# duckietown/gym-duckietown

Hardware: NVIDIA H100
Metric: env-steps/sec (obs+reward+done) at N envs, 1/2/4/8 H100 vs CPU ref (higher is better)
Workload: dtype f64 logic / f32 raster / u8 obs

## Files before the change

### gym-duckietown_b200/csrc/dts_render.cu

```cuda
#include <cstddef>

#include "dts_camera.cuh"
#include "dts_kernels.h"

namespace dts {

namespace {

#ifndef DTS_STATS
#define DTS_STATS 0
#endif
#if DTS_STATS
#define DTS_COUNT(slot, n) do { if (lane == 0) atomicAdd(err + (slot), (n)); } while (0)
#else
#define DTS_COUNT(slot, n) do { } while (0)
#endif
constexpr int kThreads = 256;
constexpr int kRasterMinCtas = 3;
constexpr int kSoloMinCtas = 3;
constexpr int kFlatMinCtas = 4;
constexpr int kGeoWarps = 1;
constexpr int kGeoMinCtas = 32;
constexpr int kWarps = kThreads / 32;
constexpr int kBinW = 8, kBinH = 4;
// ... 419 lines not shown
        if (e + lo < 0) inside &= ~(1u << f);
      }
    }
  }
  int tiny = 0;
  if (!fb && !quad && live) {
    const int minx = min(qx[0], min(qx[1], qx[2])) - ox, maxx = max(qx[0], max(qx[1], qx[2])) - ox;
    const int miny = min(qy[0], min(qy[1], qy[2])) - oy, maxy = max(qy[0], max(qy[1], qy[2])) - oy;
    const int x0 = max(minx >> 6, 0), x1 = min(maxx >> 6, kCoarseW - 1), y0 = max(miny >> 6, 0), y1 = min(maxy >> 6, kCoarseH - 1);
    if (x1 - x0 < 4 && y1 - y0 < 4 && x1 >= x0 && y1 >= y0) {
      tiny = kKindTiny;
      E0[3] = x0 | (y0 << 16); A[3] = x1 | (y1 << 16);
    }
  }
  const int id = __float_as_int(w2.w);
  int4* o = reinterpret_cast<int4*>(out);
  o[0] = make_int4(E0[0], E0[1], E0[2], E0[3]);
  o[1] = make_int4(A[0], A[1], A[2], A[3]);
  o[2] = make_int4(B[0], B[1], B[2], B[3]);
  o[3] = make_int4(__float_as_int(w2.x), __float_as_int(w2.y), __float_as_int(w2.z), id);
  o[4] = make_int4(qx[0] - ox, qy[0] - oy, (int)((unsigned)p | (live << 16) | ((inside & live) << 24)),
                   (quad ? kKindQuad : 0) | (id < 2 ? kKindGround : 0) | tiny | flat);
  return (inside & live) | (id < 2 ? kRecGround : 0u) | ((flat || id < 2) && !tiny ? kRecFlatOk : 0u);
}

struct ShadeIn {
  const PrimRec* pr;
  int x0, y0;
  float q0, qx, qy, u0, ux, uy, v0, vx, vy, r0;
  int ltq;
  unsigned tex;
};
__device__ __forceinline__ ShadeIn load_shade(const PrimRec* __restrict__ prims, unsigned w) {
  const PrimRec* pr = prims + w;
  const int2 xy0 = __ldg(reinterpret_cast<const int2*>(pr));
  const float4 w3 = __ldg(reinterpret_cast<const float4*>(pr) + 3);
  const float4 w4 = __ldg(reinterpret_cast<const float4*>(pr) + 4);
  const float4 w5 = __ldg(reinterpret_cast<const float4*>(pr) + 5);
  ShadeIn si;
  si.pr = pr; si.x0 = xy0.x; si.y0 = xy0.y;
  si.q0 = w3.x; si.qx = w3.y; si.qy = w3.z; si.u0 = w3.w;
  si.ux = w4.x; si.uy = w4.y; si.v0 = w4.z; si.vx = w4.w;
  si.vy = w5.x; si.ltq = __float_as_int(w5.y); si.tex = __float_as_uint(w5.z); si.r0 = w5.w;
  return si;
}
__device__ __forceinline__ void shade_eval(const ShadeIn& si, const uint8_t* __restrict__ tex_pool, const float4* __restrict__ lat_tab,
                                           int pxa, int pya, float c3[3]) {
  const float cdx = (float)(pxa + 32 - si.x0) * 0.015625f, cdy = (float)(pya + 32 - si.y0) * 0.015625f;
  float qq = fmaf(si.qy, cdy, fmaf(si.qx, cdx, si.q0));
  if (!(qq > 1e-20f)) qq = 1e-20f;
  const float rq = 1.0f / qq;
  const float u = fmaf(si.uy, cdy, fmaf(si.ux, cdx, si.u0)) * rq;
  const float v = fmaf(si.vy, cdy, fmaf(si.vx, cdx, si.v0)) * rq;
  const int ltq = si.ltq;
  const int lat = (ltq & 0xffff) - 1;
  if (lat >= 0) {
    const float fa_ = u * 7.0f, fb_ = (1.0f - v) * 7.0f;
    int ia = __float2int_rd(fa_), ib = __float2int_rd(fb_);
    ia = ia < 0 ? 0 : (ia > 6 ? 6 : ia);
    ib = ib < 0 ? 0 : (ib > 6 ? 6 : ib);
    const float fa = fa_ - (float)ia, fb = fb_ - (float)ib;
    const float4* L = lat_tab + lat * 64 + ia * 8 + ib;
    const bool lower = fb <= fa;
    const float4 c00 = L[0], c11 = L[9], cm = L[lower ? 8 : 1];
    const float t1 = lower ? fa : fb, t2 = lower ? fb : fa;
    c3[0] = fmaf(t2, c11.x - cm.x, fmaf(t1, cm.x - c00.x, c00.x));
    c3[1] = fmaf(t2, c11.y - cm.y, fmaf(t1, cm.y - c00.y, c00.y));
    c3[2] = fmaf(t2, c11.z - cm.z, fmaf(t1, cm.z - c00.z, c00.z));
  } else {
    const float4 w6 = __ldg(reinterpret_cast<const float4*>(si.pr) + 6);
    const float4 w7 = __ldg(reinterpret_cast<const float4*>(si.pr) + 7);
    c3[0] = fmaf(w6.y, cdy, fmaf(w6.x, cdx, si.r0)) * rq;
    c3[1] = fmaf(w7.x, cdy, fmaf(w6.w, cdx, w6.z)) * rq;
    c3[2] = fmaf(w7.w, cdy, fmaf(w7.z, cdx, w7.y)) * rq;
  }
  if (ltq & 0x00ff0000) {
    const unsigned ti = si.tex;
    const int lw = (ti >> 24) & 15, lh = ti >> 28;
    const int tw = 1 << lw, th = 1 << lh;
    const float twf = __int_as_float((127 + lw) << 23), thf = __int_as_float((127 + lh) << 23);
    const float tx = u * twf - 0.5f, ty = v * thf - 0.5f;
    const int txi = __float2int_rd(tx), tyi = __float2int_rd(ty);
    const float ffx = tx - (float)txi, ffy = ty - (float)tyi;
    const int ti0 = txi & (tw - 1), ti1 = (ti0 + 1) & (tw - 1);
    const int tj0 = tyi & (th - 1), tj1 = (tj0 + 1) & (th - 1);
    const uchar4* tp = reinterpret_cast<const uchar4*>(tex_pool + ((size_t)(ti & 0xffffffu) << 8));
    const uchar4 t00 = __ldg(tp + (tj0 << lw) + ti0), t10 = __ldg(tp + (tj0 << lw) + ti1);
    const uchar4 t01 = __ldg(tp + (tj1 << lw) + ti0), t11 = __ldg(tp + (tj1 << lw) + ti1);
    const float a0[3] = {(float)t00.x, (float)t00.y, (float)t00.z}, a1[3] = {(float)t10.x, (float)t10.y, (float)t10.z};
    const float b0[3] = {(float)t01.x, (float)t01.y, (float)t01.z}, b1[3] = {(float)t11.x, (float)t11.y, (float)t11.z};
#pragma unroll
    for (int ch = 0; ch < 3; ch++) {
      const float ta = fmaf(ffx, a1[ch] - a0[ch], a0[ch]);
      const float tb = fmaf(ffx, b1[ch] - b0[ch], b0[ch]);
      const float tc = fmaf(ffy, tb - ta, ta);
      c3[ch] = tc * (c3[ch] * 0.00392156862745098f);
    }
  }
}
__device__ __forceinline__ void shade_prim(const PrimRec* __restrict__ prims, unsigned w, const uint8_t* __restrict__ tex_pool,
                                           const float4* __restrict__ lat_tab, int pxa, int pya, float c3[3]) {
  const ShadeIn si = load_shade(prims, w);
  shade_eval(si, tex_pool, lat_tab, pxa, pya, c3);
}

__device__ __forceinline__ uint32_t smem_u32(const void* p) { return (uint32_t)__cvta_generic_to_shared(p); }
__device__ __forceinline__ void mbar_init(uint64_t* bar, int count) {
  asm volatile("mbarrier.init.shared::cta.b64 [%0], %1;" ::"r"(smem_u32(bar)), "r"(count) : "memory");
}
__device__ __forceinline__ void mbar_fence_init() {
  asm volatile("fence.mbarrier_init.release.cluster;" ::: "memory");
  asm volatile("fence.proxy.async.shared::cta;" ::: "memory");
}
__device__ __forceinline__ void mbar_expect_tx(uint64_t* bar, uint32_t bytes) {
  asm volatile("mbarrier.arrive.expect_tx.shared::cta.b64 _, [%0], %1;" ::"r"(smem_u32(bar)), "r"(bytes) : "memory");
}
__device__ __forceinline__ void bulk_load(void* dst_smem, const void* src_gmem, uint32_t bytes, uint64_t* bar) {
  asm volatile("cp.async.bulk.shared::cluster.global.mbarrier::complete_tx::bytes [%0], [%1], %2, [%3];" ::"r"(smem_u32(dst_smem)),
               "l"(src_gmem), "r"(bytes), "r"(smem_u32(bar))
               : "memory");
}
__device__ __forceinline__ void mbar_wait(uint64_t* bar, uint32_t parity) {
  uint32_t ok;
  do {
    asm volatile("{\n .reg .pred p;\n mbarrier.try_wait.parity.shared::cta.b64 p, [%1], %2;\n selp.u32 %0, 1, 0, p;\n}"
                 : "=r"(ok)
                 : "r"(smem_u32(bar)), "r"(parity)
                 : "memory");
  } while (!ok);
}

__device__ __forceinline__ unsigned pack_rgb(float r, float g, float b) {
  const unsigned ur = min(__float2uint_rn(r * 255.0f), 255u);
  const unsigned ug = min(__float2uint_rn(g * 255.0f), 255u);
  const unsigned ub = min(__float2uint_rn(b * 255.0f), 255u);
  return ur | (ug << 8) | (ub << 16);
}

struct StoreLane {
  int src_lo, src_hi;
  int sh8;
  int off;
  int j, row;
};
__device__ __forceinline__ StoreLane make_store_lane(int lane, int W) {
  StoreLane sl;
  const int j = lane & 7, rowbase = lane & ~7;
  const int p0 = (4 * j) / 3;
  sl.sh8 = (4 * j - 3 * p0) * 8;
  sl.src_lo = rowbase + min(p0, 7);
  sl.src_hi = rowbase + min(p0 + 1, 7);
  sl.off = (lane >> 3) * W * 3 + 4 * j;
  sl.j = j; sl.row = lane >> 3;
  return sl;
}
__device__ __forceinline__ void store_bin_fast(uint8_t* __restrict__ bin0, const StoreLane& sl, unsigned rgb, int rows_ok) {
  const unsigned lo = __shfl_sync(0xffffffffu, rgb, sl.src_lo);
  const unsigned hi = __shfl_sync(0xffffffffu, rgb, sl.src_hi);
  const unsigned word = __funnelshift_r(lo | (hi << 24), hi >> 8, sl.sh8);
  if (sl.j < 6 && sl.row < rows_ok) *reinterpret_cast<unsigned*>(bin0 + sl.off) = word;
}
__device__ __forceinline__ void store_bin(uint8_t* __restrict__ out, unsigned rgb, int lane, int bx, int by, int W, int H) {
  const int gx = bx * kBinW + (lane & 7), gy = by * kBinH + (lane >> 3);
  if ((W & 3) == 0 && bx * kBinW + kBinW <= W) {
    const int j = lane & 7, rowbase = lane & ~7;
    const int p0 = (4 * j) / 3, sh8 = (4 * j - 3 * p0) * 8;
    const unsigned lo = __shfl_sync(0xffffffffu, rgb, rowbase + min(p0, 7));
    const unsigned hi = __shfl_sync(0xffffffffu, rgb, rowbase + min(p0 + 1, 7));
    const unsigned long long both = (unsigned long long)lo | ((unsigned long long)hi << 24);
    if (j < 6 && gy < H)
      *reinterpret_cast<unsigned*>(out + ((size_t)gy * W + bx * kBinW) * 3 + 4 * j) = (unsigned)(both >> sh8);
// ... 559 lines not shown
        const int slot = atomicAdd(fm.work + kWorkSoloList, 1);
        fm.solo[slot] = make_uint2((unsigned)env, (unsigned)b | ((unsigned)p << 16));
        atomicOr(&no_flat[b], 1);
      }
      if (!(r & kRecFlatOk)) atomicOr(&no_flat[b], 1);
    }
  }
  if (!lean_fmt) return;
  __syncthreads();
  for (int b0 = wib * 32; b0 < cbins; b0 += nthr) {
    const int b = b0 + lane, c = b < cbins ? (cnt[b] & kCountMask) : 0;
    const bool flat = c >= 1 && c <= kStage && !no_flat[b];
    const unsigned m = __ballot_sync(0xffffffffu, flat);
    if (!m) continue;
    int base = 0;
    if (lane == 0) base = atomicAdd(fm.work + kWorkFlatList, __popc(m));
    base = __shfl_sync(0xffffffffu, base, 0);
    if (flat) {
      fm.bin_count[(size_t)env * cbins + b] = kFlatBin;
      fm.flat[base + __popc(m & ((1u << lane) - 1u))] = make_uint2((unsigned)env, (unsigned)b | ((unsigned)c << 16));
    }
  }
}

__device__ __noinline__ void emit_general(uint8_t* __restrict__ out, const GatherTab& gt, int n_peers, size_t env_off, int out_fmt,
                                          unsigned rgb, int lane, int bx, int by, int W, int H) {
  store_bin_any(out, out_fmt, rgb, lane, bx, by, W, H);
  for (int p = 0; p < n_peers; p++) store_bin_any(gt.base[p] + env_off, out_fmt, rgb, lane, bx, by, W, H);
}
__device__ __noinline__ void gather_rows_out(const uint8_t* __restrict__ src, const GatherTab& gt, size_t off, size_t nbytes, int lane) {
  __syncwarp();
  const uint8_t* s = src + off;
  if (((reinterpret_cast<size_t>(s) | nbytes) & 15) == 0) {
    bool aligned = true;
    for (int p = 0; p < gt.n; p++) aligned &= (reinterpret_cast<size_t>(gt.base[p] + off) & 15) == 0;
    if (aligned) {
      for (size_t i = (size_t)lane * 16; i < nbytes; i += 512) {
        const int4 v = __ldcg(reinterpret_cast<const int4*>(s + i));
        for (int p = 0; p < gt.n; p++) *reinterpret_cast<int4*>(gt.base[p] + off + i) = v;
      }
      return;
    }
  }
  for (size_t i = lane; i < nbytes; i += 32) {
    const uint8_t v = __ldcg(s + i);
    for (int p = 0; p < gt.n; p++) gt.base[p][off + i] = v;
  }
}

constexpr size_t kRasterSmem = (sizeof(BinRec) * 2 * kStage + 16 + 128 * sizeof(unsigned long long)) * kWarps;
__device__ __forceinline__ unsigned float_key(float f) { const unsigned b = __float_as_uint(f); return b ^ ((b >> 31) ? 0xffffffffu : 0x80000000u); }
__device__ __forceinline__ float key_float(unsigned k) { return __uint_as_float(k ^ ((k >> 31) ? 0x80000000u : 0xffffffffu)); }

__device__ __forceinline__ int sample_mask(const BinRec& br, int pxc, int pyc) {
  const int4 E = *reinterpret_cast<const int4*>(br.E0);
  const int4 A = *reinterpret_cast<const int4*>(br.A);
  const int4 B = *reinterpret_cast<const int4*>(br.B);
  const int ec0 = E.x + A.x * pxc + B.x * pyc;
  const int ec1 = E.y + A.y * pxc + B.y * pyc;
  const int ec2 = E.z + A.z * pxc + B.z * pyc;
  int mask = 0;
  if (br.kind & kKindQuad) {
    const int ec3 = E.w + A.w * pxc + B.w * pyc;
#pragma unroll
    for (int s = 0; s < 4; s++) {
      const int e0 = ec0 + A.x * sample_x(s) + B.x * sample_y(s);
      const int e1 = ec1 + A.y * sample_x(s) + B.y * sample_y(s);
      const int e2 = ec2 + A.z * sample_x(s) + B.z * sample_y(s);
      const int e3 = ec3 + A.w * sample_x(s) + B.w * sample_y(s);
      if ((e0 | e1 | e2 | e3) >= 0) mask |= 1 << s;
    }
  } else {
#pragma unroll
    for (int s = 0; s < 4; s++) {
      const int e0 = ec0 + A.x * sample_x(s) + B.x * sample_y(s);
      const int e1 = ec1 + A.y * sample_x(s) + B.y * sample_y(s);
      const int e2 = ec2 + A.z * sample_x(s) + B.z * sample_y(s);
      if ((e0 | e1 | e2) >= 0) mask |= 1 << s;
    }
  }
  return mask;
}

__device__ __forceinline__ unsigned shade_resolve(const unsigned wn[4], bool simple, const float clr[3], const PrimRec* __restrict__ prims,
                                                  const uint8_t* __restrict__ tex_pool, const float4* __restrict__ lat_tab, int pxa,
                                                  int pya, int lane, int32_t* __restrict__ err) {
  (void)lane; (void)err;
  const bool same = wn[1] == wn[0] && wn[2] == wn[0] && wn[3] == wn[0];
  const bool all_same = simple || __all_sync(0xffffffffu, same);
  float c3[3] = {clr[0], clr[1], clr[2]};
  if (wn[0] != kNoPrim) shade_prim(prims, wn[0], tex_pool, lat_tab, pxa, pya, c3);
  if (all_same) return pack_rgb(c3[0], c3[1], c3[2]);
  float s01[3] = {c3[0], c3[1], c3[2]}, s23[3] = {0.f, 0.f, 0.f};
  unsigned pend = 0xeu;
  if (wn[1] == wn[0]) { pend &= ~2u; s01[0] = s01[0] + c3[0]; s01[1] = s01[1] + c3[1]; s01[2] = s01[2] + c3[2]; }
#pragma unroll
  for (int t = 2; t < 4; t++)
    if (wn[t] == wn[0]) { pend &= ~(1u << t); s23[0] = s23[0] + c3[0]; s23[1] = s23[1] + c3[1]; s23[2] = s23[2] + c3[2]; }
#pragma unroll 1
  while (__any_sync(0xffffffffu, pend != 0u)) {
    DTS_COUNT(12, 1);
    if (pend) {
      const int s = __ffs(pend) - 1;
      const unsigned w = s == 1 ? wn[1] : (s == 2 ? wn[2] : wn[3]);
      float d3[3] = {clr[0], clr[1], clr[2]};
      if (w != kNoPrim) shade_prim(prims, w, tex_pool, lat_tab, pxa, pya, d3);
#pragma unroll
      for (int t = 1; t < 4; t++)
        if ((pend >> t & 1u) && wn[t] == w) {
          pend &= ~(1u << t);
          if (t < 2) { s01[0] = s01[0] + d3[0]; s01[1] = s01[1] + d3[1]; s01[2] = s01[2] + d3[2]; }
          else { s23[0] = s23[0] + d3[0]; s23[1] = s23[1] + d3[1]; s23[2] = s23[2] + d3[2]; }
        }
    }
  }
  return pack_rgb((s01[0] + s23[0]) * 0.25f, (s01[1] + s23[1]) * 0.25f, (s01[2] + s23[2]) * 0.25f);
}

template <bool kWrapFmt, bool kFish>
__global__ void __launch_bounds__(kThreads, kRasterMinCtas)
k_raster(const DState S, const DMap* __restrict__ maps, RenderCfg rc, FrameMem fm, FishTab ft, GatherTab gt,
         uint8_t* __restrict__ obs, int max_prims, int max_pairs, int max_lat, int32_t* __restrict__ err) {
  extern __shared__ __align__(128) unsigned char raster_smem[];
  BinRec (*stages)[2][kStage] = reinterpret_cast<BinRec (*)[2][kStage]>(raster_smem);
  uint64_t (*bars)[2] = reinterpret_cast<uint64_t (*)[2]>(raster_smem + sizeof(BinRec) * kWarps * 2 * kStage);
  unsigned long long* zb = reinterpret_cast<unsigned long long*>(raster_smem + sizeof(BinRec) * kWarps * 2 * kStage + 16 * kWarps) +
                           128 * (threadIdx.x >> 5);
  const int W = rc.width, H = rc.height;
  const int cbins_x = (W + kCoarseW - 1) / kCoarseW, cbins_y = (H + kCoarseH - 1) / kCoarseH, cbins = cbins_x * cbins_y;
  const int lane = threadIdx.x & 31, warp = threadIdx.x >> 5;
  const size_t frame_bytes = (size_t)W * H * 3;
  const int out_fmt = !kWrapFmt ? 0 : (rc.obs_layout | (rc.obs_dtype << 2));
  const size_t out_elem = (kWrapFmt && rc.obs_dtype == DTS_OBS_F32_UNIT) ? 4 : 1;
  const int pxs = (lane & 7) * kSub, pys = (lane >> 3) * kSub;
  const StoreLane sl = make_store_lane(lane, W);
  const bool fast_fmt = !kWrapFmt && lean_output(DTS_OBS_HWC, DTS_OBS_U8, W);
  const bool planar_u8 = kWrapFmt && rc.obs_dtype == DTS_OBS_U8 &&
                         ((rc.obs_layout == DTS_OBS_CHW && (W & 3) == 0) || (rc.obs_layout == DTS_OBS_CWH && (H & 3) == 0));
  uint64_t* bar = bars[warp];
  if (lane == 0) { mbar_init(&bar[0], 1); mbar_init(&bar[1], 1); mbar_fence_init(); }
  __syncwarp();
  uint32_t parity = 0;
  int cs = 0, ps = 0;
  const int n_work = rc.n_envs * cbins_y;
  int work = 0;
  if (lane == 0) work = atomicAdd(fm.work + kWorkRaster, 1);
  work = __shfl_sync(0xffffffffu, work, 0);
  while (work < n_work) {
    int next_work = 0;
    if (lane == 0) next_work = atomicAdd(fm.work + kWorkRaster, 1);
    const int env = work / cbins_y, cby = work - env * cbins_y;
    const DMap& m = maps[S.map_id[env]];
    const uint8_t* tex_pool = m.tex_pool;
    const PrimRec* prims = fm.prims + (size_t)env * max_prims;
    const BinRec* recs = fm.recs;
    const float4* lat_tab = fm.lat + (size_t)env * max_lat * 64;
    const size_t env_off = (size_t)env * frame_bytes * out_elem;
    uint8_t* out = obs + env_off;
    const bool gather_rows = gt.n > 0 && !kWrapFmt;
    auto emit = [&](unsigned rgb, int bx, int by) {
      if (fast_fmt && (gt.n == 0 || gather_rows) && bx * kBinW + kBinW <= W) {
        store_bin_fast(out + ((size_t)(by * kBinH) * W + bx * kBinW) * 3, sl, rgb, min(kBinH, H - by * kBinH));
      } else if (kWrapFmt && gt.n == 0) {
        if (planar_u8 && bx * kBinW + kBinW <= W && by * kBinH + kBinH <= H) {
          store_bin_planar_u8(out, out_fmt & 3, rgb, lane, bx, by, W, H);
        } else {
          const int gx = bx * kBinW + (lane & 7), gy = by * kBinH + (lane >> 3);
          if (gx < W && gy < H) store_px_fmt(out, out_fmt & 3, out_fmt >> 2, gx, gy, W, H, rgb);
        }
      } else {
        emit_general(out, gt, gather_rows ? 0 : gt.n, env_off, out_fmt, rgb, lane, bx, by, W, H);
      }
    };
    float clr[3];
    clear_colour(S, rc, env, clr);
    const unsigned clear_rgb = pack_rgb(clr[0], clr[1], clr[2]);
    int my_cnt = 0, my_start = 0;
    if (lane < cbins_x) {
      my_cnt = fm.bin_count[(size_t)env * cbins + cby * cbins_x + lane];
      my_start = fm.bin_start[(size_t)env * cbins + cby * cbins_x + lane];
    }
    const unsigned nz = __ballot_sync(0xffffffffu, my_cnt > 0);
    int pcbx = nz ? __ffs(nz) - 1 : 32, pf = 0, pc = 0;
    const unsigned rows_in = fine_rows_in_image(cby, H);
    auto fine_valid = [&](int cbx, int f) -> bool { return (fine_in_image(cbx, rows_in, W) >> f) & 1u; };
    auto next_bin = [&]() {
      const unsigned rem = nz & ~((2u << pcbx) - 1u);
      pcbx = rem ? __ffs(rem) - 1 : 32;
      pf = 0; pc = 0;
    };
    auto issue = [&]() {
      if (pcbx >= 32) return;
      const int n = __shfl_sync(0xffffffffu, my_cnt, pcbx), st = __shfl_sync(0xffffffffu, my_start, pcbx);
      if (n > kStage) while (pf < kCFX * kCFY && !fine_valid(pcbx, pf)) pf++;
      if (n > kStage && pf >= kCFX * kCFY) { next_bin(); return; }
      const int nch = min(kStage, n - pc);
      if (lane == 0) {
        mbar_expect_tx(&bar[ps], (uint32_t)(nch * sizeof(BinRec)));
        bulk_load(stages[warp][ps], recs + st + pc, (uint32_t)(nch * sizeof(BinRec)), &bar[ps]);
// ... 189 lines not shown
                      const int e0 = ec0 + A.x * sample_x(s) + B.x * sample_y(s);
                      const int e1 = ec1 + A.y * sample_x(s) + B.y * sample_y(s);
                      const int e2 = ec2 + A.z * sample_x(s) + B.z * sample_y(s);
                      if ((e0 | e1 | e2) < 0) continue;
                      const float sdx = (float)(X + sample_x(s) - xy0.x) * 0.015625f, sdy = (float)(Y + sample_y(s) - xy0.y) * 0.015625f;
                      const float zs = fmaf(zp.z, sdy, fmaf(zp.y, sdx, zp.x));
                      atomicMin(&zb[((py - fy0) * kBinW + (px - fx0)) * 4 + s], ((unsigned long long)float_key(zs) << 32) | tail);
                    }
                  }
              }
              __syncwarp();
            }
            if (!(last || simple)) continue;
            if (!kFish && !simple && zb_used) {
#pragma unroll
              for (int s = 0; s < 4; s++) {
                const unsigned long long k = zb[lane * 4 + s];
                if (k == ~0ull) continue;
                const float zt = key_float((unsigned)(k >> 32));
                bool win = zt < z[s];
                if (zt == z[s] && wn[s] != kNoPrim) win = (int)((k >> 16) & 0xffffu) < __ldg(&prims[wn[s]].id);
                if (win) { z[s] = zt; wn[s] = (unsigned)(k & 0xffffu); }
              }
              __syncwarp();
            }
            DTS_COUNT(11, 1);
            unsigned rgb = shade_resolve(wn, simple, clr, prims, tex_pool, lat_tab, ox + pxc, oy + pyc, lane, err);
            if (kFish && !px_valid) rgb = 0u;
            emit(rgb, bx, by);
          }
        }
      }
    }
    if (gather_rows) {
      const int rows = min(kCoarseH, H - cby * kCoarseH);
      gather_rows_out(obs, gt, env_off + (size_t)cby * kCoarseH * W * 3, (size_t)rows * W * 3, lane);
    }
    work = __shfl_sync(0xffffffffu, next_work, 0);
  }
}

template <bool kFish>
__global__ void __launch_bounds__(kThreads, kSoloMinCtas) k_raster_solo(const DState S, const DMap* __restrict__ maps, RenderCfg rc, FrameMem fm,
                                                                        FishTab ft, uint8_t* __restrict__ obs, int max_prims, int max_lat) {
  const int W = rc.width, H = rc.height;
  const int cbins_x = (W + kCoarseW - 1) / kCoarseW;
  const int lane = threadIdx.x & 31;
  const StoreLane sl = make_store_lane(lane, W);
  const size_t frame_bytes = (size_t)W * H * 3;
  const int n = fm.work[kWorkSoloList];
  const int warps = (gridDim.x * blockDim.x) >> 5;
  for (int i = (blockIdx.x * blockDim.x + threadIdx.x) >> 5; i < n; i += warps) {
    const uint2 e = fm.solo[i];
    const int env = (int)e.x, b = (int)(e.y & 0xffffu);
    const unsigned p = e.y >> 16;
    const int cby = b / cbins_x, cbx = b - cby * cbins_x;
    const uint8_t* tex_pool = maps[S.map_id[env]].tex_pool;
    const float4* lat_tab = fm.lat + (size_t)env * max_lat * 64;
    const ShadeIn si = load_shade(fm.prims + (size_t)env * max_prims, p);
    uint8_t* out = obs + (size_t)env * frame_bytes;
    const int nx = min(kCFX, (W - cbx * kCoarseW + kBinW - 1) / kBinW);
    const int ny = ((cby * kCFY + 1) * kBinH < H) ? 2 : 1;
#pragma unroll 1
    for (int fy = 0; fy < ny; fy++)
#pragma unroll 1
    for (int fx = 0; fx < nx; fx++) {
      const int bx = cbx * kCFX + fx, by = cby * kCFY + fy;
      int pxa = (bx * kBinW + (lane & 7)) * kSub, pya = (by * kBinH + (lane >> 3)) * kSub;
      bool px_valid = true;
      if (kFish) {
        const FishPx src = fish_source(ft, bx, by, lane, W, H);
        px_valid = src.valid;
        pxa = src.x; pya = src.y;
      }
      float c3[3];
      shade_eval(si, tex_pool, lat_tab, pxa, pya, c3);
      unsigned rgb = pack_rgb(c3[0], c3[1], c3[2]);
      if (kFish && !px_valid) rgb = 0u;
      store_bin_lean(out, sl, rgb, lane, bx, by, W, H);
    }
  }
}

template <bool kFish>
__global__ void __launch_bounds__(kThreads, kFlatMinCtas) k_raster_flat(const DState S, const DMap* __restrict__ maps, RenderCfg rc, FrameMem fm,
                                                                        FishTab ft, uint8_t* __restrict__ obs, int max_prims, int max_lat,
                                                                        int32_t* __restrict__ err) {
  __shared__ BinRec stages[kWarps][kStage];
  const int W = rc.width, H = rc.height;
  const int cbins_x = (W + kCoarseW - 1) / kCoarseW, cbins = cbins_x * ((H + kCoarseH - 1) / kCoarseH);
  const int lane = threadIdx.x & 31;
  BinRec* stage = stages[threadIdx.x >> 5];
  const StoreLane sl = make_store_lane(lane, W);
  const size_t frame_bytes = (size_t)W * H * 3;
  const int pxs = (lane & 7) * kSub, pys = (lane >> 3) * kSub;
  const int n = fm.work[kWorkFlatList];
  const int warps = (gridDim.x * blockDim.x) >> 5;
  for (int i = (blockIdx.x * blockDim.x + threadIdx.x) >> 5; i < n; i += warps) {
    const uint2 e = fm.flat[i];
    const int env = (int)e.x, b = (int)(e.y & 0xffffu), count = (int)(e.y >> 16);
    const int cby = b / cbins_x, cbx = b - cby * cbins_x;
    DTS_COUNT(24, 1);
    uint2 mine = make_uint2(0u, 0u);
    __syncwarp();
    if (lane < count) {
      const int4* src = reinterpret_cast<const int4*>(fm.recs + fm.bin_start[(size_t)env * cbins + b] + lane);
      int4* dst = reinterpret_cast<int4*>(stage + lane);
      int4 v[5];
#pragma unroll
      for (int k = 0; k < 5; k++) v[k] = __ldg(src + k);
#pragma unroll
      for (int k = 0; k < 5; k++) dst[k] = v[k];
      mine = make_uint2((unsigned)v[4].z, (unsigned)v[4].w);
    }
    __syncwarp();
    const unsigned ground_bits = __ballot_sync(0xffffffffu, (mine.y & kKindGround) != 0u);
    const uint8_t* tex_pool = maps[S.map_id[env]].tex_pool;
    const PrimRec* prims = fm.prims + (size_t)env * max_prims;
    const float4* lat_tab = fm.lat + (size_t)env * max_lat * 64;
    uint8_t* out = obs + (size_t)env * frame_bytes;
    float clr[3];
    clear_colour(S, rc, env, clr);
    int ox = cbx * kCoarseW * kSub, oy = cby * kCoarseH * kSub;
    if (kFish) { const short4 cb = ft.cbox[b]; ox = cb.x * kSub; oy = cb.y * kSub; }
    const int nx = min(kCFX, (W - cbx * kCoarseW + kBinW - 1) / kBinW);
    const int ny = ((cby * kCFY + 1) * kBinH < H) ? 2 : 1;
#pragma unroll 1
    for (int f = 0; f < kCFX * kCFY; f++) {
      if ((f & 3) >= nx || (f >> 2) >= ny) continue;
      const int bx = cbx * kCFX + (f & 3), by = cby * kCFY + (f >> 2);
      int pxc = pxs + (f & 3) * kBinW * kSub, pyc = pys + (f >> 2) * kBinH * kSub;
      bool px_valid = true;
      if (kFish) {
        const FishPx src = fish_source(ft, bx, by, lane, W, H);
        px_valid = src.valid;
        pxc = src.x - ox; pyc = src.y - oy;
      }
      const bool live = (mine.x >> (16 + f)) & 1u;
      const unsigned live_mask = __ballot_sync(0xffffffffu, live);
      const unsigned full_mask = __ballot_sync(0xffffffffu, live && ((mine.x >> (24 + f)) & 1u));
      const unsigned ground_mask = live_mask & ground_bits, tiles = live_mask & ~ground_mask;
      const unsigned pick = tiles ? tiles : live_mask;
      const bool simple = pick && !(pick & (pick - 1)) && (pick & full_mask);
      unsigned wn[4] = {kNoPrim, kNoPrim, kNoPrim, kNoPrim};
      if (simple) {
        const unsigned w = stage[__ffs(pick) - 1].prim_flags & 0xffffu;
        wn[0] = w; wn[1] = w; wn[2] = w; wn[3] = w;
      } else {
        int seen = 0, twice = 0;
        for (unsigned todo = tiles; todo; todo &= todo - 1) {
          const BinRec& br = stage[__ffs(todo) - 1];
          const uint32_t pflags = br.prim_flags;
          const int mask = ((pflags >> (24 + f)) & 1u) ? 15 : sample_mask(br, pxc, pyc);
          twice |= seen & mask;
          seen |= mask;
#pragma unroll
          for (int s = 0; s < 4; s++)
            if (mask >> s & 1) wn[s] = pflags & 0xffffu;
        }
        unsigned todo = __all_sync(0xffffffffu, seen == 15) ? 0u : ground_mask;
        for (; todo; todo &= todo - 1) {
          const BinRec& br = stage[__ffs(todo) - 1];
          const uint32_t pflags = br.prim_flags;
          const int mask = (((pflags >> (24 + f)) & 1u) ? 15 : sample_mask(br, pxc, pyc)) & ~(seen & 15);
          if (!mask) continue;
          twice |= (seen >> 4) & mask;
          seen |= mask << 4;
          const float4 zp = *reinterpret_cast<const float4*>(&br.z0);
          const int2 xy0 = *reinterpret_cast<const int2*>(&br.x0);
          const float cdx = (float)(pxc + 32 - xy0.x) * 0.015625f, cdy = (float)(pyc + 32 - xy0.y) * 0.015625f;
#pragma unroll
          for (int s = 0; s < 4; s++) {
            const float sdx = cdx + (float)(sample_x(s) - 32) * 0.015625f, sdy = cdy + (float)(sample_y(s) - 32) * 0.015625f;
            if ((mask >> s & 1) && fmaf(zp.z, sdy, fmaf(zp.y, sdx, zp.x)) < 1.0f) wn[s] = pflags & 0xffffu;
          }
        }
        if (__any_sync(0xffffffffu, twice != 0)) {
          DTS_COUNT(25, 1);
          if (lane == 0) fm.bin_count[(size_t)env * cbins + b] = count;
          break;
        }
      }
      unsigned rgb = shade_resolve(wn, simple, clr, prims, tex_pool, lat_tab, ox + pxc, oy + pyc, lane, err);
      if (kFish && !px_valid) rgb = 0u;
      store_bin_lean(out, sl, rgb, lane, bx, by, W, H);
    }
  }
}

__global__ void __launch_bounds__(256) k_resize(const uint8_t* __restrict__ src, int W, int H, int ow, int oh, int n_envs,
                                                const int16_t* __restrict__ xtab ,
                                                const int16_t* __restrict__ ytab , void* __restrict__ dst, int layout,
                                                int dtype) {
  const size_t total = (size_t)n_envs * ow * oh;
  for (size_t g = blockIdx.x * (size_t)blockDim.x + threadIdx.x; g < total; g += (size_t)gridDim.x * blockDim.x) {
    const int x = (int)(g % ow), y = (int)((g / ow) % oh);
    const size_t env = g / ((size_t)ow * oh);
    const int4 xa = __ldg(reinterpret_cast<const int4*>(xtab + 8 * x)), ya = __ldg(reinterpret_cast<const int4*>(ytab + 8 * y));
    const int xi[4] = {(short)(xa.x & 0xffff), xa.x >> 16, (short)(xa.y & 0xffff), xa.y >> 16};
    const int xw[4] = {(short)(xa.z & 0xffff), xa.z >> 16, (short)(xa.w & 0xffff), xa.w >> 16};
    const int yi[4] = {(short)(ya.x & 0xffff), ya.x >> 16, (short)(ya.y & 0xffff), ya.y >> 16};
    const int yw[4] = {(short)(ya.z & 0xffff), ya.z >> 16, (short)(ya.w & 0xffff), ya.w >> 16};
    const uint8_t* frame = src + env * (size_t)W * H * 3;
    long long acc[3] = {0, 0, 0};
#pragma unroll
    for (int r = 0; r < 4; r++) {
      const uint8_t* row = frame + (size_t)yi[r] * W * 3;
      int h0 = 0, h1 = 0, h2 = 0;
#pragma unroll
      for (int c = 0; c < 4; c++) {
        const uint8_t* px = row + xi[c] * 3;
        h0 += (int)px[0] * xw[c]; h1 += (int)px[1] * xw[c]; h2 += (int)px[2] * xw[c];
      }
      acc[0] += (long long)h0 * yw[r]; acc[1] += (long long)h1 * yw[r]; acc[2] += (long long)h2 * yw[r];
    }
    unsigned rgb = 0;
#pragma unroll
    for (int ch = 0; ch < 3; ch++) {
      long long v = (acc[ch] + (1LL << 21)) >> 22;
      v = v < 0 ? 0 : (v > 255 ? 255 : v);
      rgb |= (unsigned)v << (8 * ch);
    }
    void* out = reinterpret_cast<uint8_t*>(dst) + env * (size_t)ow * oh * 3 * (dtype == DTS_OBS_F32_UNIT ? 4 : 1);
    store_px_fmt(out, layout, dtype, x, y, ow, oh, rgb);
  }
}

__global__ void __launch_bounds__(256) k_blend4(const uint8_t* __restrict__ f0, const uint8_t* __restrict__ f1,
                                                const uint8_t* __restrict__ f2, const uint8_t* __restrict__ f3, double w0,
                                                double w1, double w2, double w3, double scl, double* __restrict__ out, size_t n) {
  for (size_t i = blockIdx.x * (size_t)blockDim.x + threadIdx.x; i < n; i += (size_t)gridDim.x * blockDim.x) {
    double a = (double)f0[i] * w0;
    a = a + (double)f1[i] * w1;
    a = a + (double)f2[i] * w2;
    a = a + (double)f3[i] * w3;
    out[i] = a / scl;
  }
}
static size_t device_sms() {
  int dev = 0, sms = 0;
  cudaGetDevice(&dev);
  cudaDeviceGetAttribute(&sms, cudaDevAttrMultiProcessorCount, dev);
  return sms > 0 ? (size_t)sms : 1;
}

void launch_blend4(const uint8_t* const f[4], const double w[4], double* out, size_t n, cudaStream_t st) {
  const double scl = ((w[0] + w[1]) + w[2]) + w[3];
  const size_t blocks = (n + 255) / 256, cap = device_sms() * 32;
  k_blend4<<<(unsigned)(blocks < cap ? blocks : cap), 256, 0, st>>>(f[0], f[1], f[2], f[3], w[0], w[1], w[2], w[3], scl, out, n);
}

__global__ void __launch_bounds__(256) k_resize_band(const uint8_t* __restrict__ src, int W, int H, int ow, int oh,
                                                     const int16_t* __restrict__ xtab, const int16_t* __restrict__ ytab,
                                                     void* __restrict__ dst, int layout, int dtype, int R, int cap) {
  extern __shared__ __align__(16) unsigned char rs_smem[];
  const int bands = (oh + R - 1) / R;
  const int env = blockIdx.x / bands, r0 = (blockIdx.x - env * bands) * R, r1 = min(r0 + R, oh);
  const int s_lo = ytab[8 * r0], s_hi = ytab[8 * (r1 - 1) + 3], nrows = min(s_hi - s_lo + 1, cap);
  const int rowb = W * 3, ow3 = ow * 3;
  int4* xt = reinterpret_cast<int4*>(rs_smem);
  uint8_t* sb = rs_smem + (size_t)ow * 16;
  int* hb = reinterpret_cast<int*>(sb + (((size_t)cap * rowb + 15) & ~(size_t)15));
  const uint8_t* band = src + (size_t)env * W * H * 3 + (size_t)s_lo * rowb;
  const int nbytes = nrows * rowb;
  if ((reinterpret_cast<uintptr_t>(band) & 15) == 0 && (nbytes & 15) == 0) {
    for (int i = threadIdx.x; i < nbytes / 16; i += blockDim.x) reinterpret_cast<int4*>(sb)[i] = __ldg(reinterpret_cast<const int4*>(band) + i);
  } else {
    for (int i = threadIdx.x; i < nbytes; i += blockDim.x) sb[i] = __ldg(band + i);
// ... 182 lines not shown
```

Before: 2.393 million.

## Queue edge pixels in flat raster and resolve them in warp-compacted batches

The flat raster kernel now shades the first sample per pixel inline. Pixels whose four samples hit different primitives are pushed into a per-warp shared-memory queue, and their extra samples are resolved in full 32-lane batches. This replaces the per-bin divergent loop in which a few edge lanes kept the whole warp busy. Finished colors are staged in shared memory and written out after all bins of the coarse tile are done. It also makes the texture address math unsigned and factors the row offsets. The cost is added shared memory per block, which can lower occupancy, plus extra warp syncs and queue bookkeeping.

Measured after the change: 2.544 million (median of 6 runs). 6.3% higher.

```diff
diff --git a/gym-duckietown_b200/csrc/dts_render.cu b/gym-duckietown_b200/csrc/dts_render.cu
--- a/gym-duckietown_b200/csrc/dts_render.cu
+++ b/gym-duckietown_b200/csrc/dts_render.cu
@@ -525,11 +525,12 @@
     const float tx = u * twf - 0.5f, ty = v * thf - 0.5f;
     const int txi = __float2int_rd(tx), tyi = __float2int_rd(ty);
     const float ffx = tx - (float)txi, ffy = ty - (float)tyi;
-    const int ti0 = txi & (tw - 1), ti1 = (ti0 + 1) & (tw - 1);
-    const int tj0 = tyi & (th - 1), tj1 = (tj0 + 1) & (th - 1);
+    const unsigned ti0 = (unsigned)txi & (tw - 1), ti1 = (ti0 + 1) & (tw - 1);
+    const unsigned tj0 = (unsigned)tyi & (th - 1), tj1 = (tj0 + 1) & (th - 1);
+    const unsigned r0 = tj0 << lw, r1 = tj1 << lw;
     const uchar4* tp = reinterpret_cast<const uchar4*>(tex_pool + ((size_t)(ti & 0xffffffu) << 8));
-    const uchar4 t00 = __ldg(tp + (tj0 << lw) + ti0), t10 = __ldg(tp + (tj0 << lw) + ti1);
-    const uchar4 t01 = __ldg(tp + (tj1 << lw) + ti0), t11 = __ldg(tp + (tj1 << lw) + ti1);
+    const uchar4 t00 = __ldg(tp + (r0 + ti0)), t10 = __ldg(tp + (r0 + ti1));
+    const uchar4 t01 = __ldg(tp + (r1 + ti0)), t11 = __ldg(tp + (r1 + ti1));
     const float a0[3] = {(float)t00.x, (float)t00.y, (float)t00.z}, a1[3] = {(float)t10.x, (float)t10.y, (float)t10.z};
     const float b0[3] = {(float)t01.x, (float)t01.y, (float)t01.z}, b1[3] = {(float)t11.x, (float)t11.y, (float)t11.z};
 #pragma unroll
@@ -1255,15 +1256,10 @@
   return mask;
 }
 
-__device__ __forceinline__ unsigned shade_resolve(const unsigned wn[4], bool simple, const float clr[3], const PrimRec* __restrict__ prims,
-                                                  const uint8_t* __restrict__ tex_pool, const float4* __restrict__ lat_tab, int pxa,
-                                                  int pya, int lane, int32_t* __restrict__ err) {
+__device__ __forceinline__ void resolve_edge(const unsigned wn[4], float c3[3], const float clr[3], const PrimRec* __restrict__ prims,
+                                             const uint8_t* __restrict__ tex_pool, const float4* __restrict__ lat_tab, int pxa, int pya,
+                                             int lane, int32_t* __restrict__ err) {
   (void)lane; (void)err;
-  const bool same = wn[1] == wn[0] && wn[2] == wn[0] && wn[3] == wn[0];
-  const bool all_same = simple || __all_sync(0xffffffffu, same);
-  float c3[3] = {clr[0], clr[1], clr[2]};
-  if (wn[0] != kNoPrim) shade_prim(prims, wn[0], tex_pool, lat_tab, pxa, pya, c3);
-  if (all_same) return pack_rgb(c3[0], c3[1], c3[2]);
   float s01[3] = {c3[0], c3[1], c3[2]}, s23[3] = {0.f, 0.f, 0.f};
   unsigned pend = 0xeu;
   if (wn[1] == wn[0]) { pend &= ~2u; s01[0] = s01[0] + c3[0]; s01[1] = s01[1] + c3[1]; s01[2] = s01[2] + c3[2]; }
@@ -1287,7 +1283,18 @@
         }
     }
   }
-  return pack_rgb((s01[0] + s23[0]) * 0.25f, (s01[1] + s23[1]) * 0.25f, (s01[2] + s23[2]) * 0.25f);
+#pragma unroll
+  for (int ch = 0; ch < 3; ch++) c3[ch] = (s01[ch] + s23[ch]) * 0.25f;
+}
+__device__ __forceinline__ unsigned shade_resolve(const unsigned wn[4], bool simple, const float clr[3], const PrimRec* __restrict__ prims,
+                                                  const uint8_t* __restrict__ tex_pool, const float4* __restrict__ lat_tab, int pxa,
+                                                  int pya, int lane, int32_t* __restrict__ err) {
+  const bool same = wn[1] == wn[0] && wn[2] == wn[0] && wn[3] == wn[0];
+  const bool all_same = simple || __all_sync(0xffffffffu, same);
+  float c3[3] = {clr[0], clr[1], clr[2]};
+  if (wn[0] != kNoPrim) shade_prim(prims, wn[0], tex_pool, lat_tab, pxa, pya, c3);
+  if (!all_same) resolve_edge(wn, c3, clr, prims, tex_pool, lat_tab, pxa, pya, lane, err);
+  return pack_rgb(c3[0], c3[1], c3[2]);
 }
 
 template <bool kWrapFmt, bool kFish>
@@ -1643,21 +1650,24 @@
   }
 }
 
+constexpr int kEdgeQ = 64;
 template <bool kFish>
 __global__ void __launch_bounds__(kThreads, kFlatMinCtas) k_raster_flat(const DState S, const DMap* __restrict__ maps, RenderCfg rc, FrameMem fm,
                                                                         FishTab ft, uint8_t* __restrict__ obs, int max_prims, int max_lat,
                                                                         int32_t* __restrict__ err) {
   __shared__ BinRec stages[kWarps][kStage];
+  __shared__ unsigned bin_rgb[kWarps][kCFX * kCFY * 32];
+  __shared__ uint4 edge_q[kWarps][2][kEdgeQ];
   const int W = rc.width, H = rc.height;
   const int cbins_x = (W + kCoarseW - 1) / kCoarseW, cbins = cbins_x * ((H + kCoarseH - 1) / kCoarseH);
   const int lane = threadIdx.x & 31;
   BinRec* stage = stages[threadIdx.x >> 5];
-  const StoreLane sl = make_store_lane(lane, W);
+  unsigned* rgb_buf = bin_rgb[threadIdx.x >> 5];
+  uint4 (*q)[kEdgeQ] = edge_q[threadIdx.x >> 5];
   const size_t frame_bytes = (size_t)W * H * 3;
   const int pxs = (lane & 7) * kSub, pys = (lane >> 3) * kSub;
-  const int n = fm.work[kWorkFlatList];
   const int warps = (gridDim.x * blockDim.x) >> 5;
-  for (int i = (blockIdx.x * blockDim.x + threadIdx.x) >> 5; i < n; i += warps) {
+  for (int i = (blockIdx.x * blockDim.x + threadIdx.x) >> 5; i < __ldg(fm.work + kWorkFlatList); i += warps) {
     const uint2 e = fm.flat[i];
     const int env = (int)e.x, b = (int)(e.y & 0xffffu), count = (int)(e.y >> 16);
     const int cby = b / cbins_x, cbx = b - cby * cbins_x;
@@ -1686,8 +1696,10 @@
     if (kFish) { const short4 cb = ft.cbox[b]; ox = cb.x * kSub; oy = cb.y * kSub; }
     const int nx = min(kCFX, (W - cbx * kCoarseW + kBinW - 1) / kBinW);
     const int ny = ((cby * kCFY + 1) * kBinH < H) ? 2 : 1;
+    unsigned qs = 0;
+    int f = 0;
 #pragma unroll 1
-    for (int f = 0; f < kCFX * kCFY; f++) {
+    for (; f < kCFX * kCFY; f++) {
       if ((f & 3) >= nx || (f >> 2) >= ny) continue;
       const int bx = cbx * kCFX + (f & 3), by = cby * kCFY + (f >> 2);
       int pxc = pxs + (f & 3) * kBinW * kSub, pyc = pys + (f >> 2) * kBinH * kSub;
@@ -1742,9 +1754,49 @@
           break;
         }
       }
-      unsigned rgb = shade_resolve(wn, simple, clr, prims, tex_pool, lat_tab, ox + pxc, oy + pyc, lane, err);
-      if (kFish && !px_valid) rgb = 0u;
-      store_bin_lean(out, sl, rgb, lane, bx, by, W, H);
+      float c3[3] = {clr[0], clr[1], clr[2]};
+      if (wn[0] != kNoPrim) shade_prim(prims, wn[0], tex_pool, lat_tab, ox + pxc, oy + pyc, c3);
+      const bool edge = px_valid && !(wn[1] == wn[0] && wn[2] == wn[0] && wn[3] == wn[0]);
+      const unsigned edges = __ballot_sync(0xffffffffu, edge);
+      const unsigned slot = f * 32 + lane;
+      if (edge) {
+        const int e = (qs + __popc(edges & ((1u << lane) - 1u))) & (kEdgeQ - 1);
+        q[0][e] = make_uint4(slot, (unsigned)(ox + pxc), (unsigned)(oy + pyc), wn[0] | (wn[1] << 16));
+        q[1][e] = make_uint4(wn[2] | (wn[3] << 16), __float_as_uint(c3[0]), __float_as_uint(c3[1]), __float_as_uint(c3[2]));
+      } else {
+        rgb_buf[slot] = (kFish && !px_valid) ? 0u : pack_rgb(c3[0], c3[1], c3[2]);
+      }
+      qs += __popc(edges);
+      DTS_COUNT(26, __popc(edges));
+#pragma unroll 1
+      for (int nq = (qs & 0xffffu) - (qs >> 16); nq >= 32 || (nq > 0 && f == (ny - 1) * kCFX + nx - 1); nq = (qs & 0xffffu) - (qs >> 16)) {
+        DTS_COUNT(27, 1);
+        const int take = min(nq, 32);
+        __syncwarp();
+        unsigned qw[4] = {0u, 0u, 0u, 0u};
+        float q3[3] = {0.f, 0.f, 0.f};
+        unsigned qslot = 0u;
+        int qx = 0, qy = 0;
+        if (lane < take) {
+          const int e = ((qs >> 16) + lane) & (kEdgeQ - 1);
+          const uint4 a = q[0][e], c = q[1][e];
+          qslot = a.x; qx = (int)a.y; qy = (int)a.z;
+          qw[0] = a.w & 0xffffu; qw[1] = a.w >> 16; qw[2] = c.x & 0xffffu; qw[3] = c.x >> 16;
+          q3[0] = __uint_as_float(c.y); q3[1] = __uint_as_float(c.z); q3[2] = __uint_as_float(c.w);
+        }
+        resolve_edge(qw, q3, clr, prims, tex_pool, lat_tab, qx, qy, lane, err);
+        if (lane < take) rgb_buf[qslot] = pack_rgb(q3[0], q3[1], q3[2]);
+        qs += (unsigned)take << 16;
+        __syncwarp();
+      }
+    }
+    if (f < kCFX * kCFY) continue;
+    __syncwarp();
+    const StoreLane sl = make_store_lane(lane, W);
+#pragma unroll 1
+    for (int f = 0; f < kCFX * kCFY; f++) {
+      if ((f & 3) >= nx || (f >> 2) >= ny) continue;
+      store_bin_lean(out, sl, rgb_buf[f * 32 + lane], lane, cbx * kCFX + (f & 3), cby * kCFY + (f >> 2), W, H);
     }
   }
 }
```
